# Lingeng56/conformer-pytorch-lightning

Measured on AMD Instinct MI355X. Metric: encoder frames/sec (80-d fbank, T=1000), whole job, higher is better.
Workload: dtype bf16

## Files before the change

### conformer-pytorch-lightning_amd/attention.py

```python
import math

import torch
import torch.nn as nn

import cfm
from cfm import packing
from feedforward import _inference_only


def _sinusoid_table(max_len, d_model, dtype=torch.float32):
    rate = torch.exp(torch.arange(0, d_model, 2) * (-math.log(10000.0) / d_model))
    angle = torch.arange(max_len).unsqueeze(1) * rate
    table = torch.zeros(max_len, 1, d_model, dtype=dtype)
    table[:, 0, 0::2] = torch.sin(angle)
    table[:, 0, 1::2] = torch.cos(angle)
    return table


class _SinusoidBase(nn.Module):
    _table_dtype = torch.float32

    def __init__(self, d_model, dropout, max_len=5000):
        super().__init__()
        self.dropout = nn.Dropout(p=dropout)
# ... 87 lines not shown
        q_str, kv_sb, kv_st = (Tq * D, D), Tn * 2 * D, 2 * D

    have_cache = cache is not None and cache.dim() == 4 and cache.size(0) > 0
    old = cache.to(device=query.device, dtype=torch.float32) if have_cache else None
    Tc = old.size(2) if have_cache else 0
    Tk = Tc + Tn
    new_cache = None
    if have_cache or getattr(mod, "return_cache", True):
        new_cache = cfm.kv_cache_pack(old, k_t, v_t, (kv_sb, kv_st), (kv_sb, kv_st), B, H, Tn, dk)
    if have_cache:
        k_src, v_src = new_cache, new_cache[..., dk:]
        k_str = v_str = (H * Tk * 2 * dk, 2 * dk, Tk * 2 * dk)
    else:
        k_src, v_src = k_t, v_t
        k_str = v_str = (kv_sb, kv_st, dk)

    p, p_str = None, (0, 0)
    if relative:
        pe = pos_embed.reshape(-1, D)
        R = pe.size(0)
        if R % B != 0 or R // B not in (1, Tk):
            raise RuntimeError("pos_embed with %d rows cannot be viewed as (B=%d, 1 or Tk=%d, H, d_k) (attention.py:78)" % (R, B, Tk))
        P = R // B
        p = cfm.gemm(rows(pe), pk.pos_w, w_lo=pk.pos_w_lo, out_dtype=adt)
        p_str = (P * D, D if P > 1 else 0)

    m8, m_str = _mask_args(inputs_attn_mask, B, Tq, Tk)
    ctx = torch.empty((B * Tq, D), dtype=adt, device=query.device)
    cfm.attention(q_t, k_src, v_src, B, H, Tq, Tk, dk, q_str, k_str, v_str, ctx, p=p, p_str=p_str,
                  bias_u=pk.bias_u, bias_v=pk.bias_v, mask=m8, mask_str=m_str, mma_code=prec.w_code, split=prec.split)
    out = cfm.gemm(ctx, pk.out_w, bias=pk.out_b, w_lo=pk.out_w_lo, out_dtype=torch.float32).view(B, Tq, D)
    if new_cache is None:
        new_cache = torch.zeros((0, 0, 0, 0), dtype=torch.float32, device=query.device)
    return out.to(query.dtype), new_cache


class RelativeMultiHeadSelfAttentionModule(nn.Module):

    def __init__(self, encoder_dim, num_heads, dropout):
        super().__init__()
        self.d_k = encoder_dim // num_heads
        self.num_heads = num_heads
        self.linear_pos = nn.Linear(encoder_dim, encoder_dim, bias=False)
        self.linear_k = nn.Linear(encoder_dim, encoder_dim)
        self.linear_q = nn.Linear(encoder_dim, encoder_dim)
        self.linear_v = nn.Linear(encoder_dim, encoder_dim)
        self.linear_out = nn.Linear(encoder_dim, encoder_dim)
        self.pos_bias_u = nn.Parameter(torch.empty(num_heads, self.d_k))
# ... 28 lines not shown
```

### conformer-pytorch-lightning_amd/csrc/attention.hip

```cpp
#include "cfm_common.h"
#include "attn_common.h"

struct AttnArgs {
    const void* q;
    const void* k;
    const void* v;
    const void* p;
    const float* bias_u;
    const float* bias_v;
    const uint8_t* mask;
    void* out;
    int64_t q_sb, q_st, k_sb, k_st, k_sh, v_sb, v_st, v_sh, p_sb, p_st, m_sb, m_sq;
    int B, H, Tq, Tk, dk;
    int q_dtype, kv_dtype, p_dtype, out_dtype;
    float scale;
    float* lse;
    CfmDrop drop;
};

namespace {

template <typename HT, bool HAS_POS, bool SPLIT>
__global__ __launch_bounds__(256) void cfm_attn_kernel(const AttnArgs a) {
    constexpr int NPL = SPLIT ? 2 : 1;
// ... 181 lines not shown
#ifdef CFM_ATTN_STAMPS
__device__ long long cfm_attn_stamps[2048 * 8];
#define CFM_ASTAMP(i) do { if (threadIdx.x == 0) { const int bid_ = (blockIdx.z * gridDim.y + blockIdx.y) * gridDim.x + blockIdx.x; \
        if (bid_ < 2048) cfm_attn_stamps[bid_ * 8 + (i)] = (i) >= 6 ? wall_clock64() : clock64(); } } while (0)
#else
#define CFM_ASTAMP(i) do { } while (0)
#endif

constexpr int SK = 256;
constexpr int V2STR = 72;
constexpr int MLSTR = SK + 4;

template <typename HT, bool F32>
__device__ __forceinline__ u32x4 load_row8(const void* base, unsigned off) {
    if constexpr (F32) {
        const f32x4 a = *(const f32x4*)((const float*)base + off);
        const f32x4 b = *(const f32x4*)((const float*)base + off + 4);
        return pack8<HT>(a, b);
    } else {
        return *(const u32x4*)((const u16*)base + off);
    }
}

template <typename HT, int PMODE, bool MFULL, bool KVF32, int NWQ = 4>
__device__ __forceinline__ void attn2_body(const AttnArgs& a, const int block_x) {
    constexpr int QTL = 16 * NWQ, NTH = 64 * NWQ, NST = SK * 8 / NTH;
    __shared__ u32x4 Kl[SK * 8];
    __shared__ u32x4 Pl[PMODE == 2 ? SK * 8 : 1];
    __shared__ __attribute__((aligned(16))) u16 Vl[SK * V2STR];
    __shared__ __attribute__((aligned(16))) uint8_t Ml[(MFULL ? QTL : 1) * MLSTR];

    const int tid = threadIdx.x, lane = tid & 63;
    const int wave = __builtin_amdgcn_readfirstlane(tid >> 6);
    const int g = lane >> 4, l15 = lane & 15;
    const int nq = (a.Tq + QTL - 1) / QTL;
    const int grp = block_x / (8 * nq), rem = block_x % (8 * nq);
    const int pair = grp * 8 + rem % 8;
    if (pair >= a.B * a.H) return;
    const int b = pair / a.H, h = pair % a.H;
    const int q0 = (rem / 8) * QTL;
    const int qi = q0 + wave * 16 + l15;
    const int qc = qi < a.Tq ? qi : a.Tq - 1;
    constexpr int dk = 64;
    CFM_ASTAMP(0);
    CFM_ASTAMP(6);

    u32x4 qraw[2], praw[2];
    f32x4 bu[2][2], bv[2][2];
#pragma unroll
    for (int kk = 0; kk < 2; ++kk) {
        const int d0 = kk * 32 + g * 8;
        qraw[kk] = *(const u32x4*)((const u16*)a.q + (int64_t)b * a.q_sb + (int64_t)qc * a.q_st + h * dk + d0);
        if constexpr (PMODE != 0) {
            bu[kk][0] = *(const f32x4*)(a.bias_u + h * dk + d0); bu[kk][1] = *(const f32x4*)(a.bias_u + h * dk + d0 + 4);
            bv[kk][0] = *(const f32x4*)(a.bias_v + h * dk + d0); bv[kk][1] = *(const f32x4*)(a.bias_v + h * dk + d0 + 4);
        }
        if constexpr (PMODE == 1) praw[kk] = *(const u32x4*)((const u16*)a.p + (int64_t)b * a.p_sb + h * dk + d0);
    }
    u32x4 kr[NST], vr[NST], pr[PMODE == 2 ? NST : 1];
    using kv_t = std::conditional_t<KVF32, float, u16>;
    const kv_t* const kbase = (const kv_t*)a.k + ((int64_t)b * a.k_sb + (int64_t)h * a.k_sh);
    const kv_t* const vbase = (const kv_t*)a.v + ((int64_t)b * a.v_sb + (int64_t)h * a.v_sh);
    const u16* const pbase = PMODE == 2 ? (const u16*)a.p + ((int64_t)b * a.p_sb + (int64_t)h * dk) : nullptr;
    const unsigned kst = (unsigned)a.k_st, vst = (unsigned)a.v_st, pst = (unsigned)a.p_st;
    auto stage_load = [&](int ks) {
#pragma unroll
        for (int i = 0; i < NST; ++i) {
            const int id = i * NTH + tid;
            const int key = id >> 3, c = id & 7;
            const int kj = ks + key;
            const bool ok = kj < a.Tk;
            const unsigned kc = ok ? (unsigned)kj : 0u;
            kr[i] = load_row8<HT, KVF32>(kbase, kc * kst + c * 8);
            vr[i] = load_row8<HT, KVF32>(vbase, kc * vst + c * 8);
            if constexpr (PMODE == 2) pr[i] = *(const u32x4*)(pbase + (kc * pst + c * 8));
            if (!ok) {
                kr[i] = (u32x4){0u, 0u, 0u, 0u};
                vr[i] = (u32x4){0u, 0u, 0u, 0u};
                if constexpr (PMODE == 2) pr[i] = (u32x4){0u, 0u, 0u, 0u};
            }
        }
    };
    stage_load(0);
    CFM_ASTAMP(1);

    u32x4 qu[2], qv[2];
    float bd = 0.f;
#pragma unroll
    for (int kk = 0; kk < 2; ++kk) {
        const u32x4 raw = qraw[kk];
        const unsigned w[4] = {raw.x, raw.y, raw.z, raw.w};
        float f[8];
#pragma unroll
        for (int i = 0; i < 4; ++i) {
            f[2 * i] = HT::to_f32((u16)(w[i] & 0xffffu));
            f[2 * i + 1] = HT::to_f32((u16)(w[i] >> 16));
        }
        if constexpr (PMODE == 0) {
            qu[kk] = raw;
        } else {
            const f32x4 fa = {f[0], f[1], f[2], f[3]}, fb = {f[4], f[5], f[6], f[7]};
            qu[kk] = pack8<HT>(fa + bu[kk][0], fb + bu[kk][1]);
            qv[kk] = pack8<HT>(fa + bv[kk][0], fb + bv[kk][1]);
            if constexpr (PMODE == 1) {
                const unsigned pw[4] = {praw[kk].x, praw[kk].y, praw[kk].z, praw[kk].w}, qw[4] = {qv[kk].x, qv[kk].y, qv[kk].z, qv[kk].w};
#pragma unroll
                for (int i = 0; i < 4; ++i) {
                    bd = fmaf(HT::to_f32((u16)(qw[i] & 0xffffu)), HT::to_f32((u16)(pw[i] & 0xffffu)), bd);
                    bd = fmaf(HT::to_f32((u16)(qw[i] >> 16)), HT::to_f32((u16)(pw[i] >> 16)), bd);
                }
            }
        }
    }
    if constexpr (PMODE == 1) {
        bd += __shfl_xor(bd, 16, 64);
        bd += __shfl_xor(bd, 32, 64);
    }

    f32x4 acc_o[4];
#pragma unroll
    for (int i = 0; i < 4; ++i) acc_o[i] = (f32x4){0.f, 0.f, 0.f, 0.f};
    float m_run = -INFINITY, l_run = 0.f;

    for (int ks = 0; ks < a.Tk; ks += SK) {
        if (ks) {
            __syncthreads();
            stage_load(ks);
        }
        {
            if constexpr (!MFULL) {
                const int kj = ks + tid;
                uint8_t mv = kj < a.Tk ? 1 : 0;
                if (mv && a.mask) mv = a.mask[(int64_t)b * a.m_sb + kj] != 0;
                if (tid < SK) Ml[tid] = mv;
            } else {
#pragma unroll 4
                for (int i = 0; i < QTL; ++i) {
                    const int kj = ks + (tid < SK ? tid : SK - 1);
                    const int qr = q0 + i < a.Tq ? q0 + i : a.Tq - 1;
                    if (tid < SK) Ml[i * MLSTR + tid] = kj < a.Tk ? (a.mask[(int64_t)b * a.m_sb + (int64_t)qr * a.m_sq + kj] != 0) : 0;
// ... 10 lines not shown
        }
        __syncthreads();
        CFM_ASTAMP(2);

        f32x4 s[16];
#pragma unroll
        for (int f = 0; f < 16; ++f) {
            s[f] = (f32x4){0.f, 0.f, 0.f, 0.f};
#pragma unroll
            for (int kk = 0; kk < 2; ++kk) {
                const int idx = k_swz(f * 16 + l15, kk * 4 + g);
                s[f] = HT::mfma(Kl[idx], qu[kk], s[f]);
                if constexpr (PMODE == 2) s[f] = HT::mfma(Pl[idx], qv[kk], s[f]);
            }
        }
        float tmax = -INFINITY;
        const uint8_t* mrow = Ml + (MFULL ? (wave * 16 + l15) * MLSTR : 0) + 4 * g;
#pragma unroll
        for (int f = 0; f < 16; ++f) {
            const unsigned mb = *(const unsigned*)(mrow + f * 16);
#pragma unroll
            for (int r = 0; r < 4; ++r) {
                const bool ok = ((mb >> (8 * r)) & 0xffu) != 0;
                const float x = ok ? (s[f][r] + bd) * a.scale : -INFINITY;
                s[f][r] = x;
                tmax = fmaxf(tmax, x);
            }
        }
        tmax = fmaxf(tmax, __shfl_xor(tmax, 16, 64));
        tmax = fmaxf(tmax, __shfl_xor(tmax, 32, 64));
        const float m_new = fmaxf(m_run, tmax);
        float alpha = 1.f;
        if (m_new != -INFINITY) alpha = __expf(m_run - m_new);
        float psum = 0.f;
#pragma unroll
        for (int f = 0; f < 16; ++f)
#pragma unroll
            for (int r = 0; r < 4; ++r) {
                const float pv = (m_new == -INFINITY) ? 0.f : __expf(s[f][r] - m_new);
                s[f][r] = pv;
                psum += pv;
            }
        l_run = l_run * alpha + psum;
        m_run = m_new;
#pragma unroll
        for (int i = 0; i < 4; ++i) acc_o[i] *= alpha;
        if (a.drop.thresh) {
            const unsigned rowbase = (unsigned)(((int64_t)b * a.H + h) * a.Tq + qc) * (unsigned)a.Tk;
#pragma unroll
            for (int f = 0; f < 16; ++f)
#pragma unroll
                for (int r = 0; r < 4; ++r) s[f][r] = cfm_drop(a.drop, rowbase + (unsigned)(ks + f * 16 + g * 4 + r), s[f][r]);
        }
#pragma unroll
        for (int k2 = 0; k2 < 8; ++k2) {
            const u32x4 ph = pack8<HT>(s[2 * k2], s[2 * k2 + 1]);
            const int key0 = k2 * 32 + 4 * g;
#pragma unroll
            for (int fd = 0; fd < 4; ++fd) {
                const u16* pa = Vl + (key0 + (l15 >> 2)) * V2STR + fd * 16 + (l15 & 3) * 4;
                const s16x4 lo = __builtin_amdgcn_ds_read_tr16_b64_v4i16((s16x4 __attribute__((address_space(3)))*)(pa));
                const s16x4 hi = __builtin_amdgcn_ds_read_tr16_b64_v4i16((s16x4 __attribute__((address_space(3)))*)(pa + 16 * V2STR));
                const u32x2 lo2 = __builtin_bit_cast(u32x2, lo), hi2 = __builtin_bit_cast(u32x2, hi);
                const u32x4 vf = {lo2.x, lo2.y, hi2.x, hi2.y};
                acc_o[fd] = HT::mfma(vf, ph, acc_o[fd]);
            }
        }
    }

    CFM_ASTAMP(3);
    float l_tot = l_run + __shfl_xor(l_run, 16, 64);
    l_tot += __shfl_xor(l_tot, 32, 64);
    const float inv = l_tot > 0.f ? __builtin_amdgcn_rcpf(l_tot) : 0.f;
    if (a.lse && qi < a.Tq && g == 0) a.lse[((int64_t)b * a.H + h) * a.Tq + qi] = l_tot > 0.f ? m_run + logf(l_tot) : -INFINITY;
    if (qi < a.Tq) {
        const int64_t ob = ((int64_t)b * a.Tq + qi) * ((int64_t)a.H * dk) + (int64_t)h * dk;
#pragma unroll
        for (int fd = 0; fd < 4; ++fd) {
            const int d = fd * 16 + g * 4;
            const f32x4 o = acc_o[fd] * inv;
            if (a.out_dtype == CFM_F32)
                *(f32x4*)((float*)a.out + ob + d) = o;
            else if (a.out_dtype == CFM_BF16)
                *(u32x2*)((u16*)a.out + ob + d) = (u32x2){pack2<BF16>(o.x, o.y), pack2<BF16>(o.z, o.w)};
            else
                *(u32x2*)((u16*)a.out + ob + d) = (u32x2){pack2<F16>(o.x, o.y), pack2<F16>(o.z, o.w)};
        }
    }
    CFM_ASTAMP(4);
    CFM_ASTAMP(7);
}

template <typename HT, int PMODE, bool MFULL, bool KVF32>
__global__ __launch_bounds__(256, 2) void cfm_attn2_kernel(const AttnArgs a) {
    attn2_body<HT, PMODE, MFULL, KVF32>(a, (int)blockIdx.x);
}

template <typename HT, int PMODE>
__global__ __launch_bounds__(512, 1) void cfm_attn2_q128_kernel(const AttnArgs a) {
    attn2_body<HT, PMODE, false, false, 8>(a, (int)blockIdx.x);
}

constexpr int ATTN_GROUP_MAX = 8;
struct AttnGroupArgs {
    AttnArgs a[ATTN_GROUP_MAX];
    int first[ATTN_GROUP_MAX + 1];
    int n;
};

template <typename HT, bool MFULL>
__global__ __launch_bounds__(256, 2) void cfm_attn2_group_kernel(const AttnGroupArgs G) {
    const int b = (int)blockIdx.x;
    int idx = 0;
#pragma unroll
    for (int i = 1; i < ATTN_GROUP_MAX; ++i)
        if (i < G.n && b >= G.first[i]) idx = i;
    attn2_body<HT, 0, MFULL, false>(G.a[idx], b - G.first[idx]);
}

template <typename HT>
int launch_attn2(const AttnArgs& a, hipStream_t s, const char* name) {
    const int nq = (a.Tq + QT - 1) / QT, pairs = a.B * a.H;
    const dim3 grid((unsigned)(((pairs + 7) / 8) * 8 * nq)), block(256);
    const double flops = 4.0 * a.B * a.H * (double)a.Tq * a.Tk * a.dk;
    const double bytes = 2.0 * a.B * a.H * ((double)a.Tq * 2 + (double)a.Tk * 2) * a.dk;
    CfmProfScope prof(name, s, flops, bytes);
    const int pmode = a.p ? (a.p_st == 0 ? 1 : 2) : 0;
    const bool mfull = a.mask && a.m_sq != 0;
    const bool kvf32 = a.kv_dtype == CFM_F32;
    if (!mfull && !kvf32 && pmode != 2 && a.Tq > 64 && ((pairs + 7) / 8) * 8 * ((a.Tq + 127) / 128) >= 192) {
        const int nq8 = (a.Tq + 127) / 128;
        const dim3 grid8((unsigned)(((pairs + 7) / 8) * 8 * nq8)), block8(512);
        if (pmode == 0) CFM_LAUNCH((cfm_attn2_q128_kernel<HT, 0>), grid8, block8, 0, s, a);
        else CFM_LAUNCH((cfm_attn2_q128_kernel<HT, 1>), grid8, block8, 0, s, a);
        return cfm_launch_status(name);
    }
#define CFM_A2(PM)                                                                                       \
    do {                                                                                                 \
        if (mfull && kvf32) CFM_LAUNCH((cfm_attn2_kernel<HT, PM, true, true>), grid, block, 0, s, a);      \
        else if (mfull) CFM_LAUNCH((cfm_attn2_kernel<HT, PM, true, false>), grid, block, 0, s, a);         \
        else if (kvf32) CFM_LAUNCH((cfm_attn2_kernel<HT, PM, false, true>), grid, block, 0, s, a);         \
        else CFM_LAUNCH((cfm_attn2_kernel<HT, PM, false, false>), grid, block, 0, s, a);                   \
    } while (0)
    if (pmode == 0) CFM_A2(0);
    else if (pmode == 1) CFM_A2(1);
    else CFM_A2(2);
#undef CFM_A2
    return cfm_launch_status(name);
}

__global__ void cfm_kv_pack_kernel(const float* old_cache, int Tc, const void* k, const void* v, int dt, int64_t k_sb,
                                   int64_t k_st, int64_t v_sb, int64_t v_st, float* out, int B, int H, int Tn, int dk) {
    const int Tk = Tc + Tn;
    const int64_t n = (int64_t)B * H * Tk * 2 * dk;
    for (int64_t i = (int64_t)blockIdx.x * blockDim.x + threadIdx.x; i < n; i += (int64_t)gridDim.x * blockDim.x) {
        const int e = (int)(i % (2 * dk));
        int64_t r = i / (2 * dk);
        const int t = (int)(r % Tk);
        r /= Tk;
        const int h = (int)(r % H);
        const int b = (int)(r / H);
        float val;
        if (t < Tc) {
            val = old_cache[(((int64_t)b * H + h) * Tc + t) * (2 * dk) + e];
        } else if (e < dk) {
            val = load_as_f32(k, (int64_t)b * k_sb + (int64_t)(t - Tc) * k_st + h * dk + e, dt);
        } else {
            val = load_as_f32(v, (int64_t)b * v_sb + (int64_t)(t - Tc) * v_st + h * dk + (e - dk), dt);
        }
// ... 4 lines not shown
template <typename HT, bool SPLIT>
int launch_attn(const AttnArgs& a, bool has_pos, hipStream_t s, const char* name) {
    const dim3 grid((a.Tq + QT - 1) / QT, a.H, a.B), block(256);
    const double flops = 4.0 * a.B * a.H * (double)a.Tq * a.Tk * a.dk;
    const double bytes = 2.0 * a.B * a.H * ((double)a.Tq * 2 + (double)a.Tk * 2) * a.dk;
    CfmProfScope prof(name, s, flops, bytes);
    if (has_pos)
        CFM_LAUNCH((cfm_attn_kernel<HT, true, SPLIT>), grid, block, 0, s, a);
    else
        CFM_LAUNCH((cfm_attn_kernel<HT, false, SPLIT>), grid, block, 0, s, a);
    return cfm_launch_status(name);
}

}

static int attn_args(const cfm_attn_desc* d, AttnArgs& a, bool& fast) {
    CFM_CHECK_ARG(d && d->q && d->k && d->v && d->out, "cfm_attention: null pointer");
    CFM_CHECK_ARG(d->B > 0 && d->H > 0 && d->Tq > 0 && d->Tk > 0, "cfm_attention: empty problem");
    CFM_CHECK_ARG(d->dk > 0 && d->dk <= DKP && d->dk % 4 == 0, "cfm_attention: need dk %% 4 == 0 and dk <= 64 (dk=%d)", d->dk);
    CFM_CHECK_ARG(d->B <= 65535 && d->H <= 65535, "cfm_attention: B,H must fit a grid dimension");
    CFM_CHECK_ARG(d->mma_dtype == CFM_BF16 || d->mma_dtype == CFM_F16, "cfm_attention: mma_dtype must be bf16 or fp16");
    CFM_CHECK_ARG(!d->split || d->mma_dtype == CFM_BF16, "cfm_attention: split mode uses bf16 planes");
    CFM_CHECK_ARG(!d->p || (d->bias_u && d->bias_v), "cfm_attention: positional term needs bias_u and bias_v");
    a.q = d->q; a.k = d->k; a.v = d->v; a.p = d->p; a.bias_u = d->p ? d->bias_u : nullptr; a.bias_v = d->p ? d->bias_v : nullptr;
    a.mask = d->mask; a.out = d->out;
    a.q_sb = d->q_sb; a.q_st = d->q_st; a.k_sb = d->k_sb; a.k_st = d->k_st; a.k_sh = d->k_sh;
    a.v_sb = d->v_sb; a.v_st = d->v_st; a.v_sh = d->v_sh; a.p_sb = d->p_sb; a.p_st = d->p_st; a.m_sb = d->m_sb; a.m_sq = d->m_sq;
    a.B = d->B; a.H = d->H; a.Tq = d->Tq; a.Tk = d->Tk; a.dk = d->dk;
    a.q_dtype = d->q_dtype; a.kv_dtype = d->kv_dtype; a.p_dtype = d->p_dtype; a.out_dtype = d->out_dtype; a.scale = d->scale; a.lse = d->lse;
    CFM_CHECK_ARG(d->drop_p >= 0.f && d->drop_p < 1.f, "cfm_attention: dropout probability must be in [0, 1)");
    CFM_CHECK_ARG(d->drop_p == 0.f || (int64_t)d->B * d->H * d->Tq * d->Tk < ((int64_t)1 << 32), "cfm_attention: dropout needs fewer than 2^32 score elements");
    a.drop = cfm_make_drop(d->drop_p, d->drop_seed);
    const bool pos = d->p != nullptr;
    const bool al8 = (d->q_sb % 8 == 0) && (d->q_st % 8 == 0) && (d->k_sb % 4 == 0) && (d->k_st % 8 == 0) && (d->k_sh % 8 == 0) &&
                     (d->v_sb % 4 == 0) && (d->v_st % 8 == 0) && (d->v_sh % 8 == 0) && (!pos || ((d->p_sb % 8 == 0) && (d->p_st % 8 == 0)));
    fast = !d->split && d->dk == 64 && d->q_dtype == d->mma_dtype && (!pos || d->p_dtype == d->mma_dtype) &&
           (d->kv_dtype == d->mma_dtype || d->kv_dtype == CFM_F32) && al8 &&
           (int64_t)d->Tk * d->k_st < ((int64_t)1 << 31) && (int64_t)d->Tk * d->v_st < ((int64_t)1 << 31) && (int64_t)d->Tk * d->p_st < ((int64_t)1 << 31);
    return CFM_OK;
}

extern "C" int cfm_attention(const cfm_attn_desc* d, cfm_stream_t stream) {
    AttnArgs a;
    bool fast = false;
    if (int rc = attn_args(d, a, fast)) return rc;
    hipStream_t s = (hipStream_t)stream;
    const bool pos = d->p != nullptr;
    if (fast) {
        if (d->mma_dtype == CFM_BF16) return launch_attn2<BF16>(a, s, pos ? "attn2_rel_bf16" : "attn2_bf16");
        return launch_attn2<F16>(a, s, pos ? "attn2_rel_f16" : "attn2_f16");
    }
    if (d->split) return launch_attn<BF16, true>(a, pos, s, pos ? "attn_rel_bf16x3" : "attn_bf16x3");
    if (d->mma_dtype == CFM_BF16) return launch_attn<BF16, false>(a, pos, s, pos ? "attn_rel_bf16" : "attn_bf16");
    return launch_attn<F16, false>(a, pos, s, pos ? "attn_rel_f16" : "attn_f16");
}

extern "C" int cfm_attention_group(const cfm_attn_desc* descs, int32_t n, cfm_stream_t stream) {
    CFM_CHECK_ARG(descs && n > 0, "cfm_attention_group: no problems");
    hipStream_t s = (hipStream_t)stream;
    AttnGroupArgs G;
    bool groupable = n >= 2 && n <= ATTN_GROUP_MAX;
    bool mfull0 = false;
    int first = 0;
    double flops = 0.0, bytes = 0.0;
    for (int i = 0; i < n && groupable; ++i) {
        bool fast = false;
        if (int rc = attn_args(&descs[i], G.a[i], fast)) return rc;
        const AttnArgs& a = G.a[i];
        const bool mfull = a.mask && a.m_sq != 0;
        if (i == 0) mfull0 = mfull;
        groupable = fast && !a.p && a.kv_dtype != CFM_F32 && mfull == mfull0 && descs[i].mma_dtype == descs[0].mma_dtype;
        G.first[i] = first;
        const int nq = (a.Tq + QT - 1) / QT, pairs = a.B * a.H;
        first += ((pairs + 7) / 8) * 8 * nq;
        flops += 4.0 * a.B * a.H * (double)a.Tq * a.Tk * a.dk;
        bytes += 2.0 * a.B * a.H * ((double)a.Tq * 2 + (double)a.Tk * 2) * a.dk;
    }
    if (!groupable) {
        for (int i = 0; i < n; ++i)
            if (int rc = cfm_attention(&descs[i], stream)) return rc;
        return CFM_OK;
    }
    G.n = n;
    for (int i = n; i <= ATTN_GROUP_MAX; ++i) G.first[i] = first;
    for (int i = n; i < ATTN_GROUP_MAX; ++i) G.a[i] = G.a[0];
    const bool bf = descs[0].mma_dtype == CFM_BF16;
    CfmProfScope prof(bf ? "attn2_group_bf16" : "attn2_group_f16", s, flops, bytes);
    const dim3 grid((unsigned)first), block(256);
    if (bf && mfull0) CFM_LAUNCH((cfm_attn2_group_kernel<BF16, true>), grid, block, 0, s, G);
    else if (bf) CFM_LAUNCH((cfm_attn2_group_kernel<BF16, false>), grid, block, 0, s, G);
    else if (mfull0) CFM_LAUNCH((cfm_attn2_group_kernel<F16, true>), grid, block, 0, s, G);
    else CFM_LAUNCH((cfm_attn2_group_kernel<F16, false>), grid, block, 0, s, G);
    return cfm_launch_status("cfm_attention_group");
}
// ... 16 lines not shown
```

### conformer-pytorch-lightning_amd/csrc/encoder.cpp

```cpp
#include <math.h>

#include <stdlib.h>

#include "cfm_common.h"

namespace {

const float kEps = 1e-5f;

inline const void* eoff(const void* p, int64_t elems, int dt) { return (const char*)p + elems * cfm_elt_size(dt); }

struct Ctx {
    const cfm_layer_weights* w; const cfm_layer_scratch* s; const cfm_layer_io* io; const float* x_in; float* x_out; cfm_stream_t st;
    int M, D, FF, H, dk, adt, w_dt, Tc, Tk, P;
    bool split, has_pos, ring;
    const int32_t* len;
};

int& cin_merge_flag() {
    static int flag = getenv("CFM_CIN_MERGE") == nullptr || atoi(getenv("CFM_CIN_MERGE")) != 0;
    return flag;
}

int ffsplit_max_rows() {
// ... 2 lines not shown
}

bool taps15(const Ctx& c) { return c.io->ktaps == 15 && !c.io->causal_conv; }

#define CFM_TRY(expr) do { int rc__ = (expr); if (rc__ != CFM_OK) return rc__; } while (0)

int select_route(Ctx& c) {
    const cfm_layer_weights* w = c.w; const cfm_layer_scratch* s = c.s; const cfm_layer_io* io = c.io;
    CFM_CHECK_ARG(w && s && io && c.x_in && c.x_out, "cfm_encoder_layer_forward: null pointer");
    CFM_CHECK_ARG(io->B > 0 && io->T > 0 && io->D > 0 && io->H > 0 && io->D % io->H == 0 && io->FF > 0,
                  "cfm_encoder_layer_forward: bad dims B=%d T=%d D=%d H=%d FF=%d", io->B, io->T, io->D, io->H, io->FF);
    CFM_CHECK_ARG(io->D % 16 == 0, "cfm_encoder_layer_forward: D must be a multiple of 16 (GLU interleave)");
    CFM_CHECK_ARG(c.x_in != c.x_out, "cfm_encoder_layer_forward: x_in and x_out must differ (inputs are not mutated)");
    c.M = io->B * io->T; c.D = io->D; c.FF = io->FF; c.H = io->H; c.dk = c.D / c.H; c.adt = io->act_dtype; c.w_dt = io->w_dtype;
    c.split = io->act_dtype == CFM_F32;
    c.has_pos = io->pos_rows > 0 && w->pos_w;
    c.ring = io->kv_ring != nullptr;
    CFM_CHECK_ARG(!c.ring || (io->stream_offset && io->ring_T >= io->T && !io->attn_cache && !io->new_cache),
                  "encoder layer: the K/V ring needs stream_offset and ring_T >= T, and excludes attn_cache / new_cache");
    c.Tc = io->attn_cache ? io->cache_T : 0;
    c.Tk = c.ring ? io->ring_T : c.Tc + io->T;
    c.P = 0;
    if (c.has_pos) {
        CFM_CHECK_ARG((io->pos_embed || io->pos_proj) && (io->pos_shared || io->pos_rows % io->B == 0),
                      "encoder layer: pos_embed rows (%d) must be a multiple of B (%d)", io->pos_rows, io->B);
        c.P = io->pos_shared ? io->pos_rows : io->pos_rows / io->B;
        CFM_CHECK_ARG(!io->pos_shared || c.P == c.Tk, "encoder layer: shared positions need one row per key (%d rows, Tk=%d)", io->pos_rows, c.Tk);
        CFM_CHECK_ARG(c.P == 1 || c.P == c.Tk, "encoder layer: pos_embed gives %d rows per item, need 1 or Tk=%d (attention.py:78-88)", c.P, c.Tk);
    }
    CFM_CHECK_ARG(c.Tc == 0 || io->new_cache, "encoder layer: a KV cache input needs new_cache storage");
    CFM_CHECK_ARG(!io->after_out || (io->after_g && io->after_b), "encoder layer: after_out needs after_g / after_b");
    CFM_CHECK_ARG(!io->utt_len || (!c.ring && !io->attn_cache && !io->causal_conv && !io->pad_valid),
                  "encoder layer: utt_len (a ragged batch of whole utterances) excludes kv_ring, attn_cache, causal_conv and pad_valid");
    CFM_CHECK_ARG(!io->stream_len || (c.ring && !io->utt_len && !io->pad_valid),
                  "encoder layer: stream_len (per-stream window lengths) needs kv_ring and excludes utt_len, attn_cache and pad_valid");
    c.len = io->utt_len ? io->utt_len : io->stream_len;
    const bool chains = !c.split && w->ffm_w1f && w->ffm_w2n && w->ff_w1f && w->ff_w2n && w->qkv_wf && w->out_wf && w->pw1_wf && w->pw2_wf &&
                        cfm_rowchain_supported(c.D, c.FF);
    CFM_CHECK_ARG(!io->macaron_done || chains, "encoder layer: macaron_done needs the chain path");
    if (!chains) {
        CFM_CHECK_ARG(!c.split || (w->ffm_w1_lo && w->ffm_w2_lo && w->ff_w1_lo && w->ff_w2_lo && w->qkv_w_lo && w->out_w_lo && w->pw1_w_lo && w->pw2_w_lo &&
                                   (!c.has_pos || io->pos_proj || w->pos_w_lo)),
                      "encoder layer: split mode needs the *_lo weight planes");
        const bool fused = !c.split && w->ffm_w1f && w->ffm_w2f && w->ff_w1f && w->ff_w2f && (c.D == 144 || c.D == 256) && c.FF % 32 == 0 && c.FF <= 2048;
        return fused ? CFM_ROUTE_FUSED_FFN : CFM_ROUTE_GENERAL;
    }
    const bool alone = s->psum && !io->macaron_done && !io->next_w;
    if (alone && s->psum_splits >= 3 && c.M <= CFM_PAIR_MAX_ROWS && cfm_rowchain_pair_supported(c.D, c.FF)) return CFM_ROUTE_PAIR;
    if (alone && c.M <= ffsplit_max_rows() && cfm_ffn_split_supported(c.D, c.FF) && s->psum_splits >= c.FF / 256 && w->pw2_w && io->ktaps == 15)
// ... 9 lines not shown

int gemm(const Ctx& c, const void* A, int a_dt, int64_t lda, const void* W, const void* Wlo, const float* bias, void* C, int c_dt,
         int64_t ldc, int M, int N, int K, int act, const float* res, float alpha, const uint8_t* row_mask) {
    cfm_gemm_desc d = {};
    d.A = A; d.W = W; d.W_lo = c.split ? Wlo : nullptr; d.bias = bias; d.residual = res; d.row_mask = row_mask; d.C = C;
    d.lda = lda; d.ldc = ldc; d.ldr = ldc; d.M = M; d.N = N; d.K = K;
    d.a_dtype = a_dt; d.w_dtype = c.w_dt; d.c_dtype = c_dt; d.act = act; d.alpha = alpha;
    if (act == CFM_ACT_GLU && c.len) { d.row_len = c.len; d.row_T = c.io->T; }
    return cfm_gemm(&d, c.st);
}

int layernorm(const Ctx& c, const float* g, const float* b, void* out16, const uint8_t* row_mask) {
    return cfm_layernorm(c.x_out, g, b, nullptr, 0, nullptr, nullptr, out16, c.adt, row_mask, kEps, c.M, c.D, c.st);
}

int after_norm(const Ctx& c) {
    if (!c.io->after_out) return CFM_OK;
    return cfm_layernorm(c.x_out, c.io->after_g, c.io->after_b, c.io->after_out, CFM_F32, nullptr, nullptr, nullptr, 0, nullptr, kEps, c.M, c.D, c.st);
}

int attention(const Ctx& c, bool ring_written = false) {
    const cfm_layer_weights* w = c.w; const cfm_layer_scratch* s = c.s; const cfm_layer_io* io = c.io;
    const int D = c.D, H = c.H, dk = c.dk, adt = c.adt, Tk = c.Tk;
    if (c.has_pos && !io->pos_proj)
        CFM_TRY(gemm(c, io->pos_embed, CFM_F32, D, w->pos_w, w->pos_w_lo, nullptr, s->pos, adt, D, io->pos_rows, D, D, CFM_ACT_NONE, nullptr, 0.f, nullptr));
    const void* kq = eoff(s->qkv, D, adt);
    const void* vq = eoff(s->qkv, 2 * D, adt);
    const int64_t sb = (int64_t)io->T * 3 * D, stt = 3 * D;
    if (io->new_cache)
        CFM_TRY(cfm_kv_cache_pack(io->attn_cache, c.Tc, kq, vq, adt, sb, stt, sb, stt, io->new_cache, io->B, H, io->T, dk, c.st));
    if (c.ring && !ring_written)
        CFM_TRY(cfm_kv_ring_write(kq, vq, adt, sb, stt, sb, stt, io->kv_ring, io->stream_offset, io->stream_len, io->B, H, io->T, dk, io->ring_T, c.st));
    cfm_attn_desc a = {};
    a.q = s->qkv; a.q_sb = sb; a.q_st = stt; a.q_dtype = adt;
    if (c.ring || c.Tc > 0) {
        const float* kv = c.ring ? io->kv_ring : io->new_cache;
        a.k = kv; a.v = kv + dk; a.kv_dtype = CFM_F32;
        a.k_sb = a.v_sb = (int64_t)H * Tk * 2 * dk; a.k_sh = a.v_sh = (int64_t)Tk * 2 * dk; a.k_st = a.v_st = 2 * dk;
    } else {
        a.k = kq; a.v = vq; a.kv_dtype = adt;
        a.k_sb = a.v_sb = sb; a.k_sh = a.v_sh = dk; a.k_st = a.v_st = stt;
    }
    if (c.has_pos) {
        const int64_t pld = io->pos_proj ? io->pos_proj_ld : D;
        a.p = io->pos_proj ? io->pos_proj : s->pos; a.p_dtype = adt; a.p_sb = io->pos_shared ? 0 : (int64_t)c.P * pld; a.p_st = c.P == 1 ? 0 : pld;
        a.bias_u = w->bias_u; a.bias_v = w->bias_v;
    }
    a.mask = io->attn_mask; a.m_sb = io->am_sb; a.m_sq = io->am_sq;
    a.out = s->ctx; a.out_dtype = adt;
    a.B = io->B; a.H = H; a.Tq = io->T; a.Tk = Tk; a.dk = dk;
    a.mma_dtype = c.w_dt; a.split = c.split ? 1 : 0;
    a.scale = 1.0f / sqrtf((float)dk);
    return cfm_attention(&a, c.st);
}

int depthwise(const Ctx& c) {
    const cfm_layer_weights* w = c.w; const cfm_layer_scratch* s = c.s; const cfm_layer_io* io = c.io;
    if (!io->causal_conv)
        return cfm_dwconv_bn_silu(s->glu, c.adt, w->dw_w, w->dw_b, w->bn_scale, w->bn_shift, s->dw, c.adt, io->B, io->T, c.D, io->ktaps, c.st);
    CFM_TRY(cfm_dwconv_causal_bn_silu(s->glu, c.adt, io->conv_cache, w->dw_w, w->dw_b, w->bn_scale, w->bn_shift, s->dw, c.adt, io->B, io->T, c.D, io->ktaps, c.st));
    if (!io->conv_cache) return CFM_OK;
    return cfm_conv_cache_update(s->glu, c.adt, io->conv_cache, io->stream_len, io->B, io->T, c.D, io->ktaps, c.st);
}

cfm_rowchain_desc chain(const Ctx& c, float alpha) {
    cfm_rowchain_desc d = {};
    d.M = c.M; d.D = c.D; d.FF = c.FF; d.w_dtype = c.w_dt; d.alpha = alpha; d.eps = kEps;
    return d;
}

// ... 233 lines not shown
```

### conformer-pytorch-lightning_amd/encoder.py

```python
import torch
import torch.nn as nn

import cfm
from cfm import packing
from attention import PositionalEncoding, RelativePositionalEncoding
from convolution import ConvolutionSubSampling
from encoder_layer import ConformerEncoderLayer
from utils import make_attn_mask, make_pad_mask

_NO_MASK = torch.ones((0, 0, 0))


class ConformerEncoder(nn.Module):

    def __init__(self, input_dim, kernel_size, encoder_dim, dropout, attention_dropout, pos_enc_dropout, hidden_dim,
                 num_heads, encoder_num_layers, cmvn=None, max_len=5000, use_relative=False, use_dynamic_chunk_size=False,
                 use_dynamic_left_chunk=False, static_chunk_size=-1):
        super().__init__()
        pe_cls = RelativePositionalEncoding if use_relative else PositionalEncoding
        self.position_encoding = pe_cls(encoder_dim, pos_enc_dropout, max_len)
        self.embed = ConvolutionSubSampling(input_dim=input_dim, output_dim=encoder_dim, pos_enc=self.position_encoding)
        self.encoders = nn.ModuleList([
            ConformerEncoderLayer(encoder_dim, kernel_size, dropout, attention_dropout, hidden_dim, num_heads, use_relative)
            for _ in range(encoder_num_layers)])
        self.encoder_dim = encoder_dim
        self.after_norm = nn.LayerNorm(encoder_dim, eps=1e-5)
        self.global_cmvn = cmvn
        self.use_dynamic_chunk_size = use_dynamic_chunk_size
        self.use_dynamic_left_chunk = use_dynamic_left_chunk
        self.static_chunk_size = static_chunk_size

    def _run_blocks(self, x, attn_mask, pos_embed, pad_mask, caches, keep_from, pos_shared=False, proj=None, ring=None, conv=None, streaming=False, utt_len=None, stream_len=None):
        n = len(self.encoders)
        if proj is None:
            proj = self._project_positions(pos_embed, x)
        bufs = [torch.empty_like(x), torch.empty_like(x)]
        new_caches = [] if caches is not None else None
        cur, ready = x, False
        prec = cfm.resolve_precision(self)
        fuse_after = (cfm.rowchain_supported(self.encoder_dim, self.encoders[0].hidden_dim, prec) and
                      self.after_norm.weight.dtype == torch.float32 and self.after_norm.eps == 1e-5)
        y_after = torch.empty_like(x) if fuse_after else None
        import encoder_layer as _el
        e0 = self.encoders[0]
        chain = (_el.CHAIN_BLOCKS and fuse_after and caches is None and conv is None and self.encoder_dim == 256 and
                 e0.hidden_dim == 2048 and e0.kernel_size == 15 and not getattr(e0.conv_module, "causal", False) and
                 all(b.chain_ready(prec) for b in self.encoders) and
                 not (streaming and _el.SPLIT_FFN_FEW_ROWS and _el.split_rows(x.size(0) * x.size(1), self.encoder_dim, e0.hidden_dim)))
        for i, block in enumerate(self.encoders):
            nxt = self.encoders[i + 1].norm_ff_macaron if i + 1 < n else None
            cache_i = None
            if caches is not None and caches.dim() == 5 and caches.size(0) > 0:
                cache_i = caches[i]
            elif caches is not None and caches.dim() == 4 and caches.size(0) > 0:
                cache_i = caches[i:i + 1]
            pp = None if proj is None else (proj[:, i * self.encoder_dim:], proj.stride(0))
            out, nc = block.fused_forward(cur, attn_mask, pos_embed, pad_mask, cache_i, xn_ready=ready, next_norm=nxt,
                                          out=bufs[i & 1], want_cache=caches is not None, pos_proj=pp, pos_shared=pos_shared,
# ... 3 lines not shown
                                          after=(self.after_norm.weight.detach(), self.after_norm.bias.detach(), y_after)
                                          if fuse_after and i + 1 == n else None)
            if new_caches is not None:
                new_caches.append(nc[:, :, keep_from:, :])
            cur, ready = out, nxt is not None
        if fuse_after:
            return y_after, new_caches
        y, _ = cfm.layernorm(cur.view(-1, cur.size(-1)), self.after_norm.weight.detach(), self.after_norm.bias.detach(),
                             eps=self.after_norm.eps)
        return y.view_as(cur), new_caches

    def _cmvn_args(self, inputs):
        m = self.global_cmvn
        if m is None:
            return inputs, None
        mean, istd = getattr(m, "mean", None), getattr(m, "istd", None)
        ok = (isinstance(mean, torch.Tensor) and isinstance(istd, torch.Tensor) and mean.dtype == torch.float32 and istd.dtype == torch.float32 and
              mean.dim() == 1 and mean.shape == istd.shape and mean.numel() == inputs.size(-1) and mean.device == inputs.device and
              inputs.dtype == torch.float32)
        if not ok:
            return m(inputs), None
        return inputs, (mean.contiguous(), istd.contiguous() if getattr(m, "norm_var", True) else None)

    def _project_positions(self, pos_embed, x):
        if not isinstance(self.position_encoding, RelativePositionalEncoding) or pos_embed is None:
            return None
        prec = cfm.resolve_precision(self)
        ws = [blk.self_attn.linear_pos.weight for blk in self.encoders]
        pk = packing.slot(self, "_pos_pack", packing.PackCache).get(ws, prec, lambda: packing.Packed(w=packing.matrix(torch.cat([w.detach() for w in ws], 0), prec)))
        pe = pos_embed.reshape(-1, self.encoder_dim)
        pe = (pe if pe.dtype == torch.float32 else pe.float()).contiguous()
        return cfm.gemm(pe, pk.w[0], w_lo=pk.w[1], out_dtype=prec.act_dtype)

    def set_precision(self, name):
        prec = None if name is None else (name if isinstance(name, cfm.Precision) else cfm.Precision(name))
        for m in self.modules():
            m.precision = prec
        return self

    def forward(self, inputs, input_lengths, decoding_chunk_size=0, num_decoding_chunk_size=-1):
        if self.training:
            return self.forward_window([(inputs, input_lengths)], decoding_chunk_size, num_decoding_chunk_size)[0]
        inputs, cmvn = self._cmvn_args(inputs)
        cfm.require_hip(inputs, input_lengths)
        frames = inputs.size(1)
        x = self.embed.embed_frames(inputs, cmvn)
        x, pos_embed = self.position_encoding(x, 0)
        pad_mask = cfm.valid_mask(input_lengths, x.size(1), first=6, stride=4).unsqueeze(1)
# ... 363 lines not shown
```

Baseline: 27.16 million.

## Drop broadcast positional term in inference attention and use exp2 softmax

Result: faster. 27.54 million, median of 6 (+1.4%).

```diff
diff --git a/conformer-pytorch-lightning_amd/attention.py b/conformer-pytorch-lightning_amd/attention.py
--- a/conformer-pytorch-lightning_amd/attention.py
+++ b/conformer-pytorch-lightning_amd/attention.py
@@ -133,8 +133,9 @@
         if R % B != 0 or R // B not in (1, Tk):
             raise RuntimeError("pos_embed with %d rows cannot be viewed as (B=%d, 1 or Tk=%d, H, d_k) (attention.py:78)" % (R, B, Tk))
         P = R // B
-        p = cfm.gemm(rows(pe), pk.pos_w, w_lo=pk.pos_w_lo, out_dtype=adt)
-        p_str = (P * D, D if P > 1 else 0)
+        if P > 1:
+            p = cfm.gemm(rows(pe), pk.pos_w, w_lo=pk.pos_w_lo, out_dtype=adt)
+            p_str = (P * D, D)
 
     m8, m_str = _mask_args(inputs_attn_mask, B, Tq, Tk)
     ctx = torch.empty((B * Tq, D), dtype=adt, device=query.device)
diff --git a/conformer-pytorch-lightning_amd/csrc/attention.hip b/conformer-pytorch-lightning_amd/csrc/attention.hip
--- a/conformer-pytorch-lightning_amd/csrc/attention.hip
+++ b/conformer-pytorch-lightning_amd/csrc/attention.hip
@@ -227,7 +227,7 @@
     }
 }
 
-template <typename HT, int PMODE, bool MFULL, bool KVF32, int NWQ = 4>
+template <typename HT, int PMODE, bool MFULL, bool KVF32, int NWQ = 4, bool EXP2 = false>
 __device__ __forceinline__ void attn2_body(const AttnArgs& a, const int block_x) {
     constexpr int QTL = 16 * NWQ, NTH = 64 * NWQ, NST = SK * 8 / NTH;
     __shared__ u32x4 Kl[SK * 8];
@@ -250,6 +250,8 @@
     CFM_ASTAMP(0);
     CFM_ASTAMP(6);
 
+    constexpr bool BD = PMODE == 1 && !EXP2;
+    constexpr bool QV = PMODE == 2 || BD;
     u32x4 qraw[2], praw[2];
     f32x4 bu[2][2], bv[2][2];
 #pragma unroll
@@ -258,9 +260,11 @@
         qraw[kk] = *(const u32x4*)((const u16*)a.q + (int64_t)b * a.q_sb + (int64_t)qc * a.q_st + h * dk + d0);
         if constexpr (PMODE != 0) {
             bu[kk][0] = *(const f32x4*)(a.bias_u + h * dk + d0); bu[kk][1] = *(const f32x4*)(a.bias_u + h * dk + d0 + 4);
+        }
+        if constexpr (QV) {
             bv[kk][0] = *(const f32x4*)(a.bias_v + h * dk + d0); bv[kk][1] = *(const f32x4*)(a.bias_v + h * dk + d0 + 4);
         }
-        if constexpr (PMODE == 1) praw[kk] = *(const u32x4*)((const u16*)a.p + (int64_t)b * a.p_sb + h * dk + d0);
+        if constexpr (BD) praw[kk] = *(const u32x4*)((const u16*)a.p + (int64_t)b * a.p_sb + h * dk + d0);
     }
     u32x4 kr[NST], vr[NST], pr[PMODE == 2 ? NST : 1];
     using kv_t = std::conditional_t<KVF32, float, u16>;
@@ -289,7 +293,7 @@
     stage_load(0);
     CFM_ASTAMP(1);
 
-    u32x4 qu[2], qv[2];
+    u32x4 qu[2], qv[QV ? 2 : 1];
     float bd = 0.f;
 #pragma unroll
     for (int kk = 0; kk < 2; ++kk) {
@@ -306,8 +310,8 @@
         } else {
             const f32x4 fa = {f[0], f[1], f[2], f[3]}, fb = {f[4], f[5], f[6], f[7]};
             qu[kk] = pack8<HT>(fa + bu[kk][0], fb + bu[kk][1]);
-            qv[kk] = pack8<HT>(fa + bv[kk][0], fb + bv[kk][1]);
-            if constexpr (PMODE == 1) {
+            if constexpr (QV) qv[kk] = pack8<HT>(fa + bv[kk][0], fb + bv[kk][1]);
+            if constexpr (BD) {
                 const unsigned pw[4] = {praw[kk].x, praw[kk].y, praw[kk].z, praw[kk].w}, qw[4] = {qv[kk].x, qv[kk].y, qv[kk].z, qv[kk].w};
 #pragma unroll
                 for (int i = 0; i < 4; ++i) {
@@ -317,10 +321,11 @@
             }
         }
     }
-    if constexpr (PMODE == 1) {
+    if constexpr (BD) {
         bd += __shfl_xor(bd, 16, 64);
         bd += __shfl_xor(bd, 32, 64);
     }
+    const float c2 = a.scale * 1.44269504088896341f;
 
     f32x4 acc_o[4];
 #pragma unroll
@@ -377,30 +382,45 @@
 #pragma unroll
             for (int r = 0; r < 4; ++r) {
                 const bool ok = ((mb >> (8 * r)) & 0xffu) != 0;
-                const float x = ok ? (s[f][r] + bd) * a.scale : -INFINITY;
+                float x;
+                if constexpr (EXP2) x = ok ? s[f][r] : -INFINITY;
+                else x = ok ? (s[f][r] + bd) * a.scale : -INFINITY;
                 s[f][r] = x;
                 tmax = fmaxf(tmax, x);
             }
         }
         tmax = fmaxf(tmax, __shfl_xor(tmax, 16, 64));
         tmax = fmaxf(tmax, __shfl_xor(tmax, 32, 64));
-        const float m_new = fmaxf(m_run, tmax);
+        const float m_new = fmaxf(m_run, EXP2 ? tmax * c2 : tmax);
         float alpha = 1.f;
-        if (m_new != -INFINITY) alpha = __expf(m_run - m_new);
         float psum = 0.f;
-#pragma unroll
-        for (int f = 0; f < 16; ++f)
-#pragma unroll
-            for (int r = 0; r < 4; ++r) {
-                const float pv = (m_new == -INFINITY) ? 0.f : __expf(s[f][r] - m_new);
-                s[f][r] = pv;
-                psum += pv;
-            }
+        if constexpr (EXP2) {
+            if (m_new != -INFINITY) alpha = __builtin_amdgcn_exp2f(m_run - m_new);
+            const float nm = (m_new == -INFINITY) ? 0.f : -m_new;
+#pragma unroll
+            for (int f = 0; f < 16; ++f)
+#pragma unroll
+                for (int r = 0; r < 4; ++r) {
+                    const float pv = __builtin_amdgcn_exp2f(fmaf(s[f][r], c2, nm));
+                    s[f][r] = pv;
+                    psum += pv;
+                }
+        } else {
+            if (m_new != -INFINITY) alpha = __expf(m_run - m_new);
+#pragma unroll
+            for (int f = 0; f < 16; ++f)
+#pragma unroll
+                for (int r = 0; r < 4; ++r) {
+                    const float pv = (m_new == -INFINITY) ? 0.f : __expf(s[f][r] - m_new);
+                    s[f][r] = pv;
+                    psum += pv;
+                }
+        }
         l_run = l_run * alpha + psum;
         m_run = m_new;
 #pragma unroll
         for (int i = 0; i < 4; ++i) acc_o[i] *= alpha;
-        if (a.drop.thresh) {
+        if (!EXP2 && a.drop.thresh) {
             const unsigned rowbase = (unsigned)(((int64_t)b * a.H + h) * a.Tq + qc) * (unsigned)a.Tk;
 #pragma unroll
             for (int f = 0; f < 16; ++f)
@@ -427,7 +447,7 @@
     float l_tot = l_run + __shfl_xor(l_run, 16, 64);
     l_tot += __shfl_xor(l_tot, 32, 64);
     const float inv = l_tot > 0.f ? __builtin_amdgcn_rcpf(l_tot) : 0.f;
-    if (a.lse && qi < a.Tq && g == 0) a.lse[((int64_t)b * a.H + h) * a.Tq + qi] = l_tot > 0.f ? m_run + logf(l_tot) : -INFINITY;
+    if (!EXP2 && a.lse && qi < a.Tq && g == 0) a.lse[((int64_t)b * a.H + h) * a.Tq + qi] = l_tot > 0.f ? m_run + logf(l_tot) : -INFINITY;
     if (qi < a.Tq) {
         const int64_t ob = ((int64_t)b * a.Tq + qi) * ((int64_t)a.H * dk) + (int64_t)h * dk;
 #pragma unroll
@@ -446,14 +466,14 @@
     CFM_ASTAMP(7);
 }
 
-template <typename HT, int PMODE, bool MFULL, bool KVF32>
+template <typename HT, int PMODE, bool MFULL, bool KVF32, bool EXP2>
 __global__ __launch_bounds__(256, 2) void cfm_attn2_kernel(const AttnArgs a) {
-    attn2_body<HT, PMODE, MFULL, KVF32>(a, (int)blockIdx.x);
-}
-
-template <typename HT, int PMODE>
+    attn2_body<HT, PMODE, MFULL, KVF32, 4, EXP2>(a, (int)blockIdx.x);
+}
+
+template <typename HT, int PMODE, bool EXP2>
 __global__ __launch_bounds__(512, 1) void cfm_attn2_q128_kernel(const AttnArgs a) {
-    attn2_body<HT, PMODE, false, false, 8>(a, (int)blockIdx.x);
+    attn2_body<HT, PMODE, false, false, 8, EXP2>(a, (int)blockIdx.x);
 }
 
 constexpr int ATTN_GROUP_MAX = 8;
@@ -480,26 +500,35 @@
     const double flops = 4.0 * a.B * a.H * (double)a.Tq * a.Tk * a.dk;
     const double bytes = 2.0 * a.B * a.H * ((double)a.Tq * 2 + (double)a.Tk * 2) * a.dk;
     CfmProfScope prof(name, s, flops, bytes);
-    const int pmode = a.p ? (a.p_st == 0 ? 1 : 2) : 0;
+    const int pmode = a.p ? (a.p_st == 0 ? 1 : 2) : (a.bias_u ? 1 : 0);
     const bool mfull = a.mask && a.m_sq != 0;
     const bool kvf32 = a.kv_dtype == CFM_F32;
+    const bool exp2 = !a.lse && !a.drop.thresh;
     if (!mfull && !kvf32 && pmode != 2 && a.Tq > 64 && ((pairs + 7) / 8) * 8 * ((a.Tq + 127) / 128) >= 192) {
         const int nq8 = (a.Tq + 127) / 128;
         const dim3 grid8((unsigned)(((pairs + 7) / 8) * 8 * nq8)), block8(512);
-        if (pmode == 0) CFM_LAUNCH((cfm_attn2_q128_kernel<HT, 0>), grid8, block8, 0, s, a);
-        else CFM_LAUNCH((cfm_attn2_q128_kernel<HT, 1>), grid8, block8, 0, s, a);
+        if (pmode == 0 && exp2) CFM_LAUNCH((cfm_attn2_q128_kernel<HT, 0, true>), grid8, block8, 0, s, a);
+        else if (pmode == 0) CFM_LAUNCH((cfm_attn2_q128_kernel<HT, 0, false>), grid8, block8, 0, s, a);
+        else if (exp2) CFM_LAUNCH((cfm_attn2_q128_kernel<HT, 1, true>), grid8, block8, 0, s, a);
+        else CFM_LAUNCH((cfm_attn2_q128_kernel<HT, 1, false>), grid8, block8, 0, s, a);
         return cfm_launch_status(name);
     }
-#define CFM_A2(PM)                                                                                       \
-    do {                                                                                                 \
-        if (mfull && kvf32) CFM_LAUNCH((cfm_attn2_kernel<HT, PM, true, true>), grid, block, 0, s, a);      \
-        else if (mfull) CFM_LAUNCH((cfm_attn2_kernel<HT, PM, true, false>), grid, block, 0, s, a);         \
-        else if (kvf32) CFM_LAUNCH((cfm_attn2_kernel<HT, PM, false, true>), grid, block, 0, s, a);         \
-        else CFM_LAUNCH((cfm_attn2_kernel<HT, PM, false, false>), grid, block, 0, s, a);                   \
+#define CFM_A2(PM, E2)                                                                                       \
+    do {                                                                                                     \
+        if (mfull && kvf32) CFM_LAUNCH((cfm_attn2_kernel<HT, PM, true, true, E2>), grid, block, 0, s, a);      \
+        else if (mfull) CFM_LAUNCH((cfm_attn2_kernel<HT, PM, true, false, E2>), grid, block, 0, s, a);         \
+        else if (kvf32) CFM_LAUNCH((cfm_attn2_kernel<HT, PM, false, true, E2>), grid, block, 0, s, a);         \
+        else CFM_LAUNCH((cfm_attn2_kernel<HT, PM, false, false, E2>), grid, block, 0, s, a);                   \
     } while (0)
-    if (pmode == 0) CFM_A2(0);
-    else if (pmode == 1) CFM_A2(1);
-    else CFM_A2(2);
+    if (exp2) {
+        if (pmode == 0) CFM_A2(0, true);
+        else if (pmode == 1) CFM_A2(1, true);
+        else CFM_A2(2, true);
+    } else {
+        if (pmode == 0) CFM_A2(0, false);
+        else if (pmode == 1) CFM_A2(1, false);
+        else CFM_A2(2, false);
+    }
 #undef CFM_A2
     return cfm_launch_status(name);
 }
@@ -550,7 +579,11 @@
     CFM_CHECK_ARG(d->mma_dtype == CFM_BF16 || d->mma_dtype == CFM_F16, "cfm_attention: mma_dtype must be bf16 or fp16");
     CFM_CHECK_ARG(!d->split || d->mma_dtype == CFM_BF16, "cfm_attention: split mode uses bf16 planes");
     CFM_CHECK_ARG(!d->p || (d->bias_u && d->bias_v), "cfm_attention: positional term needs bias_u and bias_v");
-    a.q = d->q; a.k = d->k; a.v = d->v; a.p = d->p; a.bias_u = d->p ? d->bias_u : nullptr; a.bias_v = d->p ? d->bias_v : nullptr;
+    CFM_CHECK_ARG(d->scale > 0.f, "cfm_attention: scale must be positive");
+    const bool infer = !d->lse && d->drop_p == 0.f;
+    CFM_CHECK_ARG(d->p || !d->bias_u || infer, "cfm_attention: bias_u without p is the inference form of the broadcast positional row (no lse, no dropout)");
+    const bool keep_p = d->p && (d->p_st != 0 || !infer);
+    a.q = d->q; a.k = d->k; a.v = d->v; a.p = keep_p ? d->p : nullptr; a.bias_u = d->bias_u; a.bias_v = keep_p ? d->bias_v : nullptr;
     a.mask = d->mask; a.out = d->out;
     a.q_sb = d->q_sb; a.q_st = d->q_st; a.k_sb = d->k_sb; a.k_st = d->k_st; a.k_sh = d->k_sh;
     a.v_sb = d->v_sb; a.v_st = d->v_st; a.v_sh = d->v_sh; a.p_sb = d->p_sb; a.p_st = d->p_st; a.m_sb = d->m_sb; a.m_sq = d->m_sq;
@@ -559,7 +592,7 @@
     CFM_CHECK_ARG(d->drop_p >= 0.f && d->drop_p < 1.f, "cfm_attention: dropout probability must be in [0, 1)");
     CFM_CHECK_ARG(d->drop_p == 0.f || (int64_t)d->B * d->H * d->Tq * d->Tk < ((int64_t)1 << 32), "cfm_attention: dropout needs fewer than 2^32 score elements");
     a.drop = cfm_make_drop(d->drop_p, d->drop_seed);
-    const bool pos = d->p != nullptr;
+    const bool pos = keep_p;
     const bool al8 = (d->q_sb % 8 == 0) && (d->q_st % 8 == 0) && (d->k_sb % 4 == 0) && (d->k_st % 8 == 0) && (d->k_sh % 8 == 0) &&
                      (d->v_sb % 4 == 0) && (d->v_st % 8 == 0) && (d->v_sh % 8 == 0) && (!pos || ((d->p_sb % 8 == 0) && (d->p_st % 8 == 0)));
     fast = !d->split && d->dk == 64 && d->q_dtype == d->mma_dtype && (!pos || d->p_dtype == d->mma_dtype) &&
@@ -573,14 +606,14 @@
     bool fast = false;
     if (int rc = attn_args(d, a, fast)) return rc;
     hipStream_t s = (hipStream_t)stream;
-    const bool pos = d->p != nullptr;
+    const bool pos = a.p || a.bias_u;
     if (fast) {
         if (d->mma_dtype == CFM_BF16) return launch_attn2<BF16>(a, s, pos ? "attn2_rel_bf16" : "attn2_bf16");
         return launch_attn2<F16>(a, s, pos ? "attn2_rel_f16" : "attn2_f16");
     }
-    if (d->split) return launch_attn<BF16, true>(a, pos, s, pos ? "attn_rel_bf16x3" : "attn_bf16x3");
-    if (d->mma_dtype == CFM_BF16) return launch_attn<BF16, false>(a, pos, s, pos ? "attn_rel_bf16" : "attn_bf16");
-    return launch_attn<F16, false>(a, pos, s, pos ? "attn_rel_f16" : "attn_f16");
+    if (d->split) return launch_attn<BF16, true>(a, a.p != nullptr, s, pos ? "attn_rel_bf16x3" : "attn_bf16x3");
+    if (d->mma_dtype == CFM_BF16) return launch_attn<BF16, false>(a, a.p != nullptr, s, pos ? "attn_rel_bf16" : "attn_bf16");
+    return launch_attn<F16, false>(a, a.p != nullptr, s, pos ? "attn_rel_f16" : "attn_f16");
 }
 
 extern "C" int cfm_attention_group(const cfm_attn_desc* descs, int32_t n, cfm_stream_t stream) {
@@ -597,7 +630,7 @@
         const AttnArgs& a = G.a[i];
         const bool mfull = a.mask && a.m_sq != 0;
         if (i == 0) mfull0 = mfull;
-        groupable = fast && !a.p && a.kv_dtype != CFM_F32 && mfull == mfull0 && descs[i].mma_dtype == descs[0].mma_dtype;
+        groupable = fast && !a.p && !a.bias_u && a.kv_dtype != CFM_F32 && mfull == mfull0 && descs[i].mma_dtype == descs[0].mma_dtype;
         G.first[i] = first;
         const int nq = (a.Tq + QT - 1) / QT, pairs = a.B * a.H;
         first += ((pairs + 7) / 8) * 8 * nq;
diff --git a/conformer-pytorch-lightning_amd/csrc/encoder.cpp b/conformer-pytorch-lightning_amd/csrc/encoder.cpp
--- a/conformer-pytorch-lightning_amd/csrc/encoder.cpp
+++ b/conformer-pytorch-lightning_amd/csrc/encoder.cpp
@@ -48,9 +48,9 @@
     c.Tk = c.ring ? io->ring_T : c.Tc + io->T;
     c.P = 0;
     if (c.has_pos) {
-        CFM_CHECK_ARG((io->pos_embed || io->pos_proj) && (io->pos_shared || io->pos_rows % io->B == 0),
-                      "encoder layer: pos_embed rows (%d) must be a multiple of B (%d)", io->pos_rows, io->B);
+        CFM_CHECK_ARG(io->pos_shared || io->pos_rows % io->B == 0, "encoder layer: pos_embed rows (%d) must be a multiple of B (%d)", io->pos_rows, io->B);
         c.P = io->pos_shared ? io->pos_rows : io->pos_rows / io->B;
+        CFM_CHECK_ARG(c.P == 1 || io->pos_embed || io->pos_proj, "encoder layer: a positional table (%d rows per item) needs pos_embed or pos_proj", c.P);
         CFM_CHECK_ARG(!io->pos_shared || c.P == c.Tk, "encoder layer: shared positions need one row per key (%d rows, Tk=%d)", io->pos_rows, c.Tk);
         CFM_CHECK_ARG(c.P == 1 || c.P == c.Tk, "encoder layer: pos_embed gives %d rows per item, need 1 or Tk=%d (attention.py:78-88)", c.P, c.Tk);
     }
@@ -106,7 +106,8 @@
 int attention(const Ctx& c, bool ring_written = false) {
     const cfm_layer_weights* w = c.w; const cfm_layer_scratch* s = c.s; const cfm_layer_io* io = c.io;
     const int D = c.D, H = c.H, dk = c.dk, adt = c.adt, Tk = c.Tk;
-    if (c.has_pos && !io->pos_proj)
+    const bool table = c.has_pos && c.P != 1;
+    if (table && !io->pos_proj)
         CFM_TRY(gemm(c, io->pos_embed, CFM_F32, D, w->pos_w, w->pos_w_lo, nullptr, s->pos, adt, D, io->pos_rows, D, D, CFM_ACT_NONE, nullptr, 0.f, nullptr));
     const void* kq = eoff(s->qkv, D, adt);
     const void* vq = eoff(s->qkv, 2 * D, adt);
@@ -125,11 +126,11 @@
         a.k = kq; a.v = vq; a.kv_dtype = adt;
         a.k_sb = a.v_sb = sb; a.k_sh = a.v_sh = dk; a.k_st = a.v_st = stt;
     }
-    if (c.has_pos) {
+    if (table) {
         const int64_t pld = io->pos_proj ? io->pos_proj_ld : D;
-        a.p = io->pos_proj ? io->pos_proj : s->pos; a.p_dtype = adt; a.p_sb = io->pos_shared ? 0 : (int64_t)c.P * pld; a.p_st = c.P == 1 ? 0 : pld;
-        a.bias_u = w->bias_u; a.bias_v = w->bias_v;
-    }
+        a.p = io->pos_proj ? io->pos_proj : s->pos; a.p_dtype = adt; a.p_sb = io->pos_shared ? 0 : (int64_t)c.P * pld; a.p_st = pld;
+    }
+    if (c.has_pos) { a.bias_u = w->bias_u; a.bias_v = w->bias_v; }
     a.mask = io->attn_mask; a.m_sb = io->am_sb; a.m_sq = io->am_sq;
     a.out = s->ctx; a.out_dtype = adt;
     a.B = io->B; a.H = H; a.Tq = io->T; a.Tk = Tk; a.dk = dk;
diff --git a/conformer-pytorch-lightning_amd/encoder.py b/conformer-pytorch-lightning_amd/encoder.py
--- a/conformer-pytorch-lightning_amd/encoder.py
+++ b/conformer-pytorch-lightning_amd/encoder.py
@@ -33,7 +33,7 @@
     def _run_blocks(self, x, attn_mask, pos_embed, pad_mask, caches, keep_from, pos_shared=False, proj=None, ring=None, conv=None, streaming=False, utt_len=None, stream_len=None):
         n = len(self.encoders)
         if proj is None:
-            proj = self._project_positions(pos_embed, x)
+            proj = self._project_positions(pos_embed, x, pos_shared)
         bufs = [torch.empty_like(x), torch.empty_like(x)]
         new_caches = [] if caches is not None else None
         cur, ready = x, False
@@ -83,8 +83,10 @@
             return m(inputs), None
         return inputs, (mean.contiguous(), istd.contiguous() if getattr(m, "norm_var", True) else None)
 
-    def _project_positions(self, pos_embed, x):
+    def _project_positions(self, pos_embed, x, pos_shared=False):
         if not isinstance(self.position_encoding, RelativePositionalEncoding) or pos_embed is None:
+            return None
+        if not pos_shared and pos_embed.numel() == x.size(0) * self.encoder_dim:
             return None
         prec = cfm.resolve_precision(self)
         ws = [blk.self_attn.linear_pos.weight for blk in self.encoders]
```
